# quantscious/finmlkit

Hardware: AMD Instinct MI355X
Metric: ticks/sec aggregated to bars (higher is better)
Workload: dtype f64

## Files before the change

### finmlkit_amd/csrc/fmk_median.h

```cpp
#pragma once
#include <math.h>

#include "fmk_common.h"
#include "fmk_dpp.h"

template <bool AF64> struct MedKey;
template <> struct MedKey<false> {
    typedef uint32_t K;
    static constexpr int BITS = 32;
    static constexpr K MAXK = 0xFFFFFFFFu;
    static constexpr K KEY_NEG_INF = 0x007FFFFFu;
    static constexpr K KEY_POS_INF = 0xFF800000u;
    __device__ static __forceinline__ K tokey(K u) { return (u & 0x80000000u) ? ~u : (u | 0x80000000u); }
    __device__ static __forceinline__ K load(const void *p, int64_t j) { return tokey(((const uint32_t *)p)[j]); }
    __device__ static __forceinline__ double value(K k)
    {
        uint32_t u = (k & 0x80000000u) ? (k & 0x7FFFFFFFu) : ~k;
        return (double)__uint_as_float(u);
    }
};
template <> struct MedKey<true> {
    typedef uint64_t K;
    static constexpr int BITS = 64;
    static constexpr K MAXK = 0xFFFFFFFFFFFFFFFFull;
// ... 21 lines not shown
__device__ __forceinline__ K med_wave_umax(K v)
{
#pragma unroll
    for (int o = 32; o > 0; o >>= 1) { K w = __shfl_xor(v, o, 64); v = w > v ? w : v; }
    return v;
}

template <typename K>
__device__ __forceinline__ K med_bitonic64(K v, int lane)
{
#pragma unroll
    for (int k = 2; k <= 64; k <<= 1) {
#pragma unroll
        for (int j = k >> 1; j > 0; j >>= 1) {
            K w = __shfl_xor(v, j, 64);
            bool up = (lane & k) == 0;
            bool lower = (lane & j) == 0;
            K mn = w < v ? w : v, mx = w < v ? v : w;
            v = (lower == up) ? mn : mx;
        }
    }
    return v;
}

template <bool AF64, int NREG, bool EXACT = false>
struct MedBar {
    typedef MedKey<AF64> MK;
    typedef typename MK::K K;
    K key[NREG > 0 ? NREG : 1];
    const void *amount;
    int64_t start, cnt;
    int lane;

    __device__ __forceinline__ void load_all()
    {
        if constexpr (NREG > 0) {
            K raw[NREG];
#pragma unroll
            for (int r = 0; r < NREG; ++r) {
                const int64_t j = (int64_t)r * 64 + lane;
                raw[r] = 0;
                if (j < cnt) raw[r] = ((const K *)amount)[start + j];
            }
#pragma unroll
            for (int r = 0; r < NREG; ++r) asm volatile("" : "+v"(raw[r]));
#pragma unroll
            for (int r = 0; r < NREG; ++r) {
                const int64_t j = (int64_t)r * 64 + lane;
                key[r] = j < cnt ? MK::tokey(raw[r]) : MK::MAXK;
            }
        }
    }
    __device__ __forceinline__ bool maybe_invalid(int r) const { return !EXACT || r == NREG - 1; }
    __device__ __forceinline__ void minmax(K &mn, K &mx)
    {
        K a = MK::MAXK, b = 0;
        if constexpr (NREG > 0) {
#pragma unroll
            for (int r = 0; r < NREG; ++r) {
                const K k = key[r];
                a = k < a ? k : a;
                if (maybe_invalid(r)) b = (k != MK::MAXK && k > b) ? k : b;
                else b = k > b ? k : b;
            }
        } else {
            for (int64_t j = lane; j < cnt; j += 64) {
                K k = MK::load(amount, start + j);
                a = k < a ? k : a;
                b = k > b ? k : b;
            }
        }
        mn = med_wave_umin<K>(a);
        mx = med_wave_umax<K>(b);
    }
    __device__ __forceinline__ int64_t count_le(K pivot)
    {
        if constexpr (NREG > 0) {
            int c = 0;
#pragma unroll
            for (int r = 0; r < NREG; ++r) c += med_popc(key[r] <= pivot);
            return c;
        } else {
            int64_t c = 0;
            for (int64_t j = lane; j < cnt; j += 64) c += MK::load(amount, start + j) <= pivot;
            return fmk_wave_sum(c);
        }
    }
    __device__ __forceinline__ void split(K pivot, K &below, K &above)
    {
        K a = 0, b = MK::MAXK;
        if constexpr (NREG > 0) {
#pragma unroll
            for (int r = 0; r < NREG; ++r) {
                const K k = key[r];
                a = (k <= pivot && k > a) ? k : a;
                b = (k > pivot && k < b) ? k : b;
            }
        } else {
            for (int64_t j = lane; j < cnt; j += 64) {
                K k = MK::load(amount, start + j);
                a = (k <= pivot && k > a) ? k : a;
                b = (k > pivot && k < b) ? k : b;
            }
        }
        below = med_wave_umax<K>(a);
        above = med_wave_umin<K>(b);
    }
    __device__ __forceinline__ void inside_minmax(K lo, K hi, K &mn, K &mx)
    {
        K a = MK::MAXK, b = 0;
#pragma unroll
        for (int r = 0; r < (NREG > 0 ? NREG : 1); ++r) {
            const K k = key[r];
            const bool in = k > lo && k <= hi;
            a = (in && k < a) ? k : a;
            b = (in && k > b) ? k : b;
        }
        mn = med_wave_umin<K>(a);
        mx = med_wave_umax<K>(b);
    }
    __device__ __forceinline__ void compact(K lo, K hi, K *buf)
    {
        int base = 0;
        if constexpr (NREG > 0) {
#pragma unroll
            for (int r = 0; r < NREG; ++r) {
                K k = key[r];
                bool in = k > lo && k <= hi;
                uint64_t m = __ballot(in);
                int pos = base + __builtin_amdgcn_mbcnt_hi((uint32_t)(m >> 32), __builtin_amdgcn_mbcnt_lo((uint32_t)m, 0));
                if (in) buf[pos] = k;
                base += __popcll(m);
            }
        } else {
            for (int64_t j0 = 0; j0 < cnt; j0 += 64) {
                int64_t j = j0 + lane;
                K k = j < cnt ? MK::load(amount, start + j) : MK::MAXK;
                bool in = j < cnt && k > lo && k <= hi;
                uint64_t m = __ballot(in);
                int pos = base + __builtin_amdgcn_mbcnt_hi((uint32_t)(m >> 32), __builtin_amdgcn_mbcnt_lo((uint32_t)m, 0));
                if (in) buf[pos] = k;
                base += __popcll(m);
            }
        }
    }
};

template <bool AF64, int NREG, bool EXACT, bool SNAP = false>
__device__ __forceinline__ bool med_rank_pair(MedBar<AF64, NREG, EXACT> &bar, typename MedKey<AF64>::K *buf,
                                              int64_t k1, int64_t k2, typename MedKey<AF64>::K &v1,
                                              typename MedKey<AF64>::K &v2)
{
    typedef MedKey<AF64> MK;
    typedef typename MK::K K;
    const int lane = bar.lane;
    const int64_t cnt = bar.cnt;
    K mn, mx;
    bar.minmax(mn, mx);
    if (mn < MK::KEY_NEG_INF || mx > MK::KEY_POS_INF) return false;
    K lo = mn - 1, hi = mx;
    int64_t clo = 0, chi = cnt;
    for (int nstep = 0;; ++nstep) {
        if constexpr (SNAP && NREG > 0) {
            if (chi - clo > 64 && hi - lo > 1 && (nstep == 10 || nstep == 16 || nstep == 22)) {
                K mn_in, mx_in;
                bar.inside_minmax(lo, hi, mn_in, mx_in);
                hi = mx_in;
                lo = (mn_in == mx_in ? mx_in : mn_in) - 1;
                continue;
            }
        }
        if (chi - clo <= 64) {
            buf[lane] = MK::MAXK;
            __builtin_amdgcn_wave_barrier();
            bar.compact(lo, hi, buf);
            __builtin_amdgcn_wave_barrier();
            K v = med_bitonic64<K>(buf[lane], lane);
            __builtin_amdgcn_wave_barrier();
            v1 = __shfl(v, (int)(k1 - clo), 64);
            v2 = __shfl(v, (int)(k2 - clo), 64);
            break;
        }
        if (hi - lo == 1) { v1 = v2 = hi; break; }
        K pivot = lo + ((hi - lo) >> 1);
        int64_t c = bar.count_le(pivot);
        if (c > k2) { hi = pivot; chi = c; }
        else if (c <= k1) { lo = pivot; clo = c; }
        else {
            bar.split(pivot, v1, v2);
            break;
        }
    }
    return true;
}

template <bool AF64, int NREG, bool EXACT, bool SNAP = false>
__device__ __forceinline__ double med_search(MedBar<AF64, NREG, EXACT> &bar, typename MedKey<AF64>::K *buf)
{
    typedef MedKey<AF64> MK;
    typename MK::K v1, v2;
    const int64_t cnt = bar.cnt;
    if (!med_rank_pair<AF64, NREG, EXACT, SNAP>(bar, buf, (cnt - 1) >> 1, cnt >> 1, v1, v2)) return NAN;
    return (cnt & 1) ? MK::value(v1) : (MK::value(v1) + MK::value(v2)) / 2.0;
}

template <bool AF64, int NREG>
__device__ __forceinline__ double med_select(const void *amount, int64_t start, int64_t cnt, int lane,
                                             typename MedKey<AF64>::K *buf)
{
    MedBar<AF64, NREG, false> bar;
    bar.amount = amount; bar.start = start; bar.cnt = cnt; bar.lane = lane;
    bar.load_all();
    return med_search<AF64, NREG, false>(bar, buf);
}

#define MED_SEL_BITS 11
#define MED_SEL_BINS (1 << MED_SEL_BITS)
template <bool AF64, int THREADS>
__device__ __forceinline__ void med_block_select(const void *__restrict__ amount, int64_t start, int64_t cnt, int64_t rank0,
                                                 int64_t rank1, typename MedKey<AF64>::K &k1, typename MedKey<AF64>::K &k2,
                                                 bool &any_nan)
{
    typedef MedKey<AF64> MK;
    typedef typename MK::K K;
    constexpr int D = (MK::BITS + MED_SEL_BITS - 1) / MED_SEL_BITS;
    constexpr int PER = MED_SEL_BINS / THREADS;
    constexpr int NW = THREADS / 64;
    __shared__ unsigned hist[2][MED_SEL_BINS];
    __shared__ K s_prefix[2];
    __shared__ int64_t s_rank[2];
    __shared__ unsigned s_wsum[2][NW];
    __shared__ int s_nan;
    const int tid = threadIdx.x, lane = fmk_lane(), w = tid >> 6;
    __syncthreads();
    if (tid == 0) { s_prefix[0] = 0; s_prefix[1] = 0; s_rank[0] = rank0; s_rank[1] = rank1; s_nan = 0; }
    bool nan = false;
#pragma unroll 1
    for (int p = 0; p < D; ++p) {
#pragma unroll
        for (int q = 0; q < PER; ++q) { hist[0][tid + q * THREADS] = 0; hist[1][tid + q * THREADS] = 0; }
        __syncthreads();
        const K pre0 = s_prefix[0], pre1 = s_prefix[1];
        const int64_t rk0 = s_rank[0], rk1 = s_rank[1];
        const bool same = pre0 == pre1;
        const int rest = MK::BITS - MED_SEL_BITS * (p + 1);
        const int shift = rest > 0 ? rest : 0;
        const int width = rest >= 0 ? MED_SEL_BITS : MED_SEL_BITS + rest;
        const unsigned mask = (1u << width) - 1u;
        for (int64_t j = tid; j < cnt; j += THREADS) {
            const K k = MK::load(amount, start + j);
            if (p == 0) nan |= k < MK::KEY_NEG_INF || k > MK::KEY_POS_INF;
            const K hi = p == 0 ? (K)0 : (K)(k >> (shift + width));
            const unsigned d = (unsigned)(k >> shift) & mask;
            if (hi == pre0) atomicAdd(&hist[0][d], 1u);
            if (!same && hi == pre1) atomicAdd(&hist[1][d], 1u);
        }
        __syncthreads();
#pragma unroll
        for (int t = 0; t < 2; ++t) {
            const unsigned *hh = hist[same ? 0 : t];
            unsigned h[PER], tot = 0;
#pragma unroll
            for (int q = 0; q < PER; ++q) { h[q] = hh[tid * PER + q]; tot += h[q]; }
            unsigned inc = tot;
#pragma unroll
            for (int o = 1; o < 64; o <<= 1) { const unsigned v = __shfl_up(inc, o, 64); if (lane >= o) inc += v; }
            if (lane == 63) s_wsum[t][w] = inc;
            __syncthreads();
            unsigned base = 0;
            for (int k = 0; k < w; ++k) base += s_wsum[t][k];
            int64_t cum = (int64_t)base + inc - tot;
            const int64_t rk = t == 0 ? rk0 : rk1;
#pragma unroll
            for (int q = 0; q < PER; ++q) {
                if (cum <= rk && rk < cum + h[q]) {
                    s_prefix[t] = (K)(((t == 0 ? pre0 : pre1) << width) | (K)(tid * PER + q));
                    s_rank[t] = rk - cum;
                }
                cum += h[q];
            }
        }
        __syncthreads();
    }
    if (nan) s_nan = 1;
    __syncthreads();
    k1 = s_prefix[0]; k2 = s_prefix[1]; any_nan = s_nan != 0;
}

struct FuMed {
    uint32_t lo, hi;
    uint32_t width;
    int have;
};

__device__ __forceinline__ uint32_t fu_wave_umin(uint32_t v)
{
    return (uint32_t)fmk_dpp_reduce((int)(v ^ 0x80000000u), (int)0x7FFFFFFF, FmkOpMin()) ^ 0x80000000u;
}
__device__ __forceinline__ uint32_t fu_wave_umax(uint32_t v)
{
    return (uint32_t)fmk_dpp_reduce((int)(v ^ 0x80000000u), (int)0x80000000, FmkOpMax()) ^ 0x80000000u;
}

template <int R>
__device__ __forceinline__ double fu_median(const uint32_t (&key)[R], int cnt, int lane, bool maybe_nan, FuMed &med, uint32_t *buf)
{
    typedef MedKey<false> MK;
    const int k1 = (cnt - 1) >> 1, k2 = cnt >> 1;
    uint32_t lo = 0, hi = 0;
    int clo = 0, chi = cnt;
    bool inside = false;
    if (med.have && !maybe_nan) {
        int c1 = 0, c2 = 0;
#pragma unroll
        for (int i = 0; i < R; ++i) {
            c1 += med_popc(key[i] <= med.lo);
            c2 += med_popc(key[i] <= med.hi);
        }
        if (c1 <= k1 && k2 < c2) {
            inside = true; lo = med.lo; hi = med.hi; clo = c1; chi = c2;
            const int nc = c2 - c1;
            if (nc > 144) med.width -= med.width >> 2;
            else if (nc < 80) med.width += (med.width >> 2) + 1;
        }
    }
    if (!inside) {
        uint32_t a = MK::MAXK, bmax = 0;
#pragma unroll
        for (int i = 0; i < R; ++i) {
            const uint32_t k = key[i];
            a = k < a ? k : a;
            bmax = (k != MK::MAXK && k > bmax) ? k : bmax;
        }
        const uint32_t mn = fu_wave_umin(a), mx = fu_wave_umax(bmax);
        if (mn < MK::KEY_NEG_INF || mx > MK::KEY_POS_INF) { med.have = 0; return NAN; }
        lo = mn - 1; hi = mx; clo = 0; chi = cnt;
    }
    uint32_t v1 = 0, v2 = 0;
    bool found = false;
    while (chi - clo > 64) {
        if (hi - lo == 1) { v1 = v2 = hi; found = true; break; }
        const uint32_t pivot = lo + ((hi - lo) >> 1);
        int c = 0;
#pragma unroll
        for (int i = 0; i < R; ++i) c += med_popc(key[i] <= pivot);
        if (c > k2) { hi = pivot; chi = c; }
        else if (c <= k1) { lo = pivot; clo = c; }
        else {
            uint32_t a = 0, bb = MK::MAXK;
#pragma unroll
            for (int i = 0; i < R; ++i) {
                const uint32_t k = key[i];
                a = (k <= pivot && k > a) ? k : a;
                bb = (k > pivot && k < bb) ? k : bb;
            }
            v1 = fu_wave_umax(a); v2 = fu_wave_umin(bb);
            found = true;
            break;
        }
    }
    uint32_t cmin = 0, cmax = 0;
    if (!found) {
        buf[lane] = MK::MAXK;
        __builtin_amdgcn_wave_barrier();
        int base = 0;
#pragma unroll
        for (int i = 0; i < R; ++i) {
            const uint32_t k = key[i];
            const bool in = k > lo && k <= hi;
            const uint64_t m = __ballot(in);
            const int pos = base + (int)__builtin_amdgcn_mbcnt_hi((uint32_t)(m >> 32), __builtin_amdgcn_mbcnt_lo((uint32_t)m, 0));
            if (in) buf[pos] = k;
            base += __popcll(m);
        }
        __builtin_amdgcn_wave_barrier();
        const uint32_t c0 = buf[lane];
        __builtin_amdgcn_wave_barrier();
        if (!inside) {
            cmin = fu_wave_umin(c0);
            cmax = fu_wave_umax(lane < chi - clo ? c0 : 0u);
        }
        for (;;) {
            if (hi - lo == 1) { v1 = v2 = hi; break; }
            const uint32_t pivot = lo + ((hi - lo) >> 1);
            const int c = clo + med_popc(c0 <= pivot);
            if (c > k2) hi = pivot;
            else if (c <= k1) lo = pivot;
            else {
                v1 = fu_wave_umax(c0 <= pivot ? c0 : 0u);
                v2 = fu_wave_umin(c0 > pivot ? c0 : MK::MAXK);
                break;
            }
        }
    }
    if (!inside) {
        if (found) med.width = 64;
        else {
            const uint32_t wl = v1 - cmin, wh = cmax - v2;
            med.width = wl > wh ? wl : wh;
        }
        med.have = 1;
    }
    med.lo = v1 > med.width + 1 ? v1 - med.width - 1 : 0;
    med.hi = v2 < 0xFFFFFFFEu - med.width ? v2 + med.width : 0xFFFFFFFEu;
    return (cnt & 1) ? MK::value(v1) : (MK::value(v1) + MK::value(v2)) / 2.0;
}
```

### finmlkit_amd/csrc/fmk_ohlcv.hip

```cpp
#include <math.h>
#include <stdlib.h>

#include <utility>

#include "fmk_bars.h"
#include "fmk_common.h"
#include "fmk_dpp.h"
#include "fmk_f32tie.h"
#include "fmk_median.h"

#define FMK_SMALL_NCH 21
#define FMK_PACKED_MAX_MEAN 64

struct OhlcvOut {
    double *open, *high, *low, *close;
    float *vol;
    double *vwap;
    int64_t *trades;
    double *median;
    unsigned long long *vol_redo;
};

__device__ __forceinline__ void ohlcv_empty(const OhlcvOut &o, int64_t b, const double *price, int64_t e, int64_t n)
{
// ... 75 lines not shown
    if (go && *go == 0) return;
    __shared__ double s_red[4][OH_WIDE_THREADS / 64];
    __shared__ int s_ncand;
    __shared__ int64_t s_below[OH_WIDE_THREADS / 64];
    __shared__ int s_nan;
    const int tid = threadIdx.x, lane = fmk_lane(), w = tid >> 6;
    const int64_t n_list = list[0];
    for (int64_t q = blockIdx.x; q < n_list; q += gridDim.x) {
        const int64_t b = list[1 + q], s = ci[b], e = ci[b + 1], start = s + 1;
        double hi = -INFINITY, lo = INFINITY, tv = 0.0, td = 0.0;
        uint32_t blo = 0, bhi = 0;
        int64_t below = 0;
        bool nan = false;
        uint32_t *mycand = nullptr;
        int cap = 0;
        if constexpr (MED) {
            blo = brk[4 * q]; bhi = brk[4 * q + 1];
            mycand = cand + ((start - base) >> 2);
            cap = (int)((e - s) >> 2);
            if (tid == 0) { s_ncand = 0; s_nan = 0; }
            __syncthreads();
        }
        auto med_tick = [&](int64_t jj, bool in_bar) {
            if constexpr (MED) {
                const uint32_t raw = in_bar ? ((const uint32_t *)amount)[jj] : 0u;
                const uint32_t k = MedKey<false>::tokey(raw);
                nan |= in_bar && (k < MedKey<false>::KEY_NEG_INF || k > MedKey<false>::KEY_POS_INF);
                below += (in_bar && k < blo) ? 1 : 0;
                const bool inb = in_bar && k >= blo && k <= bhi;
                const uint64_t m = __ballot(inb);
                if (m) {
                    int base = 0;
                    if (lane == (int)__builtin_ctzll(m)) base = atomicAdd(&s_ncand, (int)__popcll(m));
                    base = __builtin_amdgcn_readlane(base, (int)__builtin_ctzll(m));
                    const int pos = base + (int)__builtin_amdgcn_mbcnt_hi((uint32_t)(m >> 32), __builtin_amdgcn_mbcnt_lo((uint32_t)m, 0));
                    if (inb && pos < cap) mycand[pos] = raw;
                }
            }
        };
        int64_t j = start + tid;
        for (; j + 3 * OH_WIDE_THREADS <= e; j += 4 * OH_WIDE_THREADS) {
            const double p0 = price[j], p1 = price[j + OH_WIDE_THREADS], p2 = price[j + 2 * OH_WIDE_THREADS],
                         p3 = price[j + 3 * OH_WIDE_THREADS];
            const double a0 = fmk_amt<AF64>(amount, j), a1 = fmk_amt<AF64>(amount, j + OH_WIDE_THREADS),
                         a2 = fmk_amt<AF64>(amount, j + 2 * OH_WIDE_THREADS), a3 = fmk_amt<AF64>(amount, j + 3 * OH_WIDE_THREADS);
            hi = fmax(fmax(hi, p0), fmax(p1, fmax(p2, p3)));
            lo = fmin(fmin(lo, p0), fmin(p1, fmin(p2, p3)));
            tv += a0; td += p0 * a0;
            tv += a1; td += p1 * a1;
            tv += a2; td += p2 * a2;
            tv += a3; td += p3 * a3;
            med_tick(j, true); med_tick(j + OH_WIDE_THREADS, true); med_tick(j + 2 * OH_WIDE_THREADS, true);
            med_tick(j + 3 * OH_WIDE_THREADS, true);
        }
        for (; j - tid <= e; j += OH_WIDE_THREADS) {
            const bool in_bar = j <= e;
            const int64_t jc = in_bar ? j : e;
            const double p0 = price[jc], a0 = in_bar ? fmk_amt<AF64>(amount, jc) : 0.0;
            hi = fmax(hi, p0);
            lo = fmin(lo, p0);
            tv += a0; td += in_bar ? p0 * a0 : 0.0;
            med_tick(jc, in_bar);
        }
        hi = fmk_dpp_reduce(hi, (double)-INFINITY, FmkOpMax());
        lo = fmk_dpp_reduce(lo, (double)INFINITY, FmkOpMin());
        tv = fmk_dpp_reduce(tv, 0.0, FmkOpAdd());
        td = fmk_dpp_reduce(td, 0.0, FmkOpAdd());
        if constexpr (MED) {
            below = fmk_dpp_reduce(below, (int64_t)0, FmkOpAdd());
            if (lane == 0) s_below[w] = below;
            if (__ballot(nan) != 0 && lane == 0) s_nan = 1;
        }
        if (lane == 0) { s_red[0][w] = hi; s_red[1][w] = lo; s_red[2][w] = tv; s_red[3][w] = td; }
        __syncthreads();
        if constexpr (MED) {
            if (tid == 0) {
                int64_t bl = 0;
                for (int k = 0; k < OH_WIDE_THREADS / 64; ++k) bl += s_below[k];
                res[3 * q] = bl; res[3 * q + 1] = s_ncand; res[3 * q + 2] = s_nan;
            }
        }
        if (w == 0) {
            hi = s_red[0][0]; lo = s_red[1][0]; tv = s_red[2][0]; td = s_red[3][0];
            for (int k = 1; k < OH_WIDE_THREADS / 64; ++k) {
                hi = fmax(hi, s_red[0][k]); lo = fmin(lo, s_red[1][k]); tv += s_red[2][k]; td += s_red[3][k];
            }
            ohlcv_finish<AF64>(o, b, price, start, e, hi, lo, tv, td, lane, true);
        }
        __syncthreads();
    }
}


struct OhlBracket { uint32_t blo, bhi; int ok; int pad; };
struct OhlCount { int64_t below; int64_t ncand; int64_t nan; };

__device__ __forceinline__ int ohl_stride(int64_t cnt) { return cnt <= 65536 ? 16 : (cnt <= ((int64_t)1 << 21) ? 64 : 256); }

__global__ __launch_bounds__(256) void k_bar_med_sample(const float *__restrict__ amount, const int64_t *__restrict__ ci,
                                                        const int64_t *__restrict__ list, const int *__restrict__ go,
                                                        float *__restrict__ samp, OhlBracket *__restrict__ brk, float g_scale,
                                                        int64_t base)
{
    if (go && *go == 0) return;
    const int64_t n_list = list[0];
    for (int64_t q = blockIdx.x; q < n_list; q += gridDim.x) {
        const int64_t b = list[1 + q], s0 = ci[b], e = ci[b + 1], start = s0 + 1, cnt = e - s0;
        const int stride = ohl_stride(cnt);
        const int64_t ns = cnt / stride;
        float *mine = samp + ((start - base) >> 4);
        for (int64_t j = threadIdx.x; j < ns; j += 256) mine[j] = amount[start + j * stride];
        __syncthreads();
        const int g = (int)(1.9f * g_scale * sqrtf((float)ns)) + 4;
        const int64_t r_lo = ns / 2 - g > 0 ? ns / 2 - g : 0, r_hi = ns / 2 + g < ns - 1 ? ns / 2 + g : ns - 1;
        uint32_t klo, khi;
        bool any_nan;
        med_block_select<false, 256>(mine, 0, ns, r_lo, r_hi, klo, khi, any_nan);
        if (threadIdx.x == 0) brk[q] = OhlBracket{klo, khi, any_nan ? 0 : 1, 0};
        __syncthreads();
    }
}

__global__ __launch_bounds__(256) void k_bar_med_finish(const int64_t *__restrict__ ci, const int64_t *__restrict__ list,
                                                        const int *__restrict__ go, const uint32_t *__restrict__ cand,
                                                        const OhlCount *__restrict__ res, int64_t *__restrict__ fallback,
                                                        double *__restrict__ o_median, int64_t base)
{
    if (go && *go == 0) return;
    typedef MedKey<false> MK;
    const int64_t n_list = list[0];
    for (int64_t q = blockIdx.x; q < n_list; q += gridDim.x) {
        const int64_t b = list[1 + q], s0 = ci[b], e = ci[b + 1], start = s0 + 1, cnt = e - s0;
        const OhlCount r = res[q];
        const int64_t k1 = (cnt - 1) >> 1, k2 = cnt >> 1, cap = cnt >> 2;
        if (r.nan) { if (threadIdx.x == 0) o_median[b] = NAN; continue; }
        if (!(r.below <= k1 && k2 < r.below + r.ncand && r.ncand <= cap)) {
            if (threadIdx.x == 0) fallback[1 + atomicAdd((unsigned long long *)fallback, 1ULL)] = b;
            continue;
        }
        uint32_t v1, v2;
        bool any_nan;
        med_block_select<false, 256>(cand + ((start - base) >> 2), 0, r.ncand, k1 - r.below, k2 - r.below, v1, v2, any_nan);
        if (threadIdx.x == 0) o_median[b] = (cnt & 1) ? MK::value(v1) : (MK::value(v1) + MK::value(v2)) / 2.0;
        __syncthreads();
    }
}

int fmk_median_long_list_launch(fmk_ctx *ctx, const void *d_amount, const int64_t *d_close_idx, const int64_t *d_list, double *d_median);

__global__ __launch_bounds__(256) void k_list_span(const int64_t *__restrict__ ci, const int64_t *__restrict__ list, int64_t *__restrict__ out)
{
    __shared__ long long s_lo, s_hi;
    if (threadIdx.x == 0) { s_lo = INT64_MAX; s_hi = 0; }
    __syncthreads();
    const int64_t n_list = list[0];
    long long lo = INT64_MAX, hi = 0;
    for (int64_t q = threadIdx.x; q < n_list; q += 256) {
        const int64_t b = list[1 + q];
        const long long s = ci[b] + 1, e = ci[b + 1] + 1;
        lo = s < lo ? s : lo;
        hi = e > hi ? e : hi;
    }
    atomicMin(&s_lo, lo);
    atomicMax(&s_hi, hi);
    __syncthreads();
    if (threadIdx.x == 0) { out[0] = n_list; out[1] = n_list ? s_lo : 0; out[2] = n_list ? s_hi : 0; }
}

template <bool AF64>
static int oh_wide_launch(fmk_ctx *ctx, const double *p, const void *a, const int64_t *ci, int64_t nb, int64_t n, const int *go,
                          const OhlcvOut &o, int *median_done = nullptr, int64_t wide_min = OH_WIDE_MIN)
{
    int64_t *list = nullptr;
    FMK_TRY(fmk_long_bar_list(ctx, ci, nb, n, wide_min, go, &list));
    if constexpr (!AF64) {
        if (o.median && median_done) {
            const int64_t cap = n / wide_min + 2;
            int64_t base = 0, span = n;
            if (!ctx->enqueue_only) {
                int64_t *d_span = ctx->d_mail->ohlcv.span, h_span[3];
                k_list_span<<<1, 256, 0, ctx->stream>>>(ci, list, d_span);
                FMK_LAUNCH_CHECK(ctx);
                FMK_TRY(fmk_read_back(ctx, h_span, d_span, sizeof h_span));
                if (h_span[0] == 0) {
                    FMK_TRY(fmk_free(ctx, list));
                    *median_done = 1;
                    return FMK_OK;
                }
                base = h_span[1] & ~(int64_t)15;
                span = h_span[2] - base;
            }
            float *samp = nullptr;
            uint32_t *cand = nullptr;
            OhlBracket *brk = nullptr;
            int64_t *res = nullptr, *fallback = nullptr;
            int rc = fmk_alloc(ctx, (size_t)((span >> 4) + 64) * 4, (void **)&samp);
            if (rc == FMK_OK) rc = fmk_alloc(ctx, (size_t)((span >> 2) + 64) * 4, (void **)&cand);
            if (rc == FMK_OK) rc = fmk_alloc(ctx, (size_t)cap * sizeof(OhlBracket), (void **)&brk);
            if (rc == FMK_OK) rc = fmk_alloc(ctx, (size_t)cap * 3 * 8, (void **)&res);
            if (rc == FMK_OK) rc = fmk_alloc(ctx, (size_t)(cap + 1) * 8, (void **)&fallback);
            const bool have_scratch = rc == FMK_OK;
            hipError_t le = hipSuccess;
            if (have_scratch) le = hipMemsetAsync(fallback, 0, 8, ctx->stream);
            if (have_scratch && le == hipSuccess) {
                const char *gv = getenv("FMK_WIDE_MED_GSCALE");
                k_bar_med_sample<<<(unsigned)(ctx->n_cu * 4), 256, 0, ctx->stream>>>((const float *)a, ci, list, go, samp, brk,
                                                                                   gv ? (float)atof(gv) : 1.0f, base);
                k_bar_ohlcv_wide<false, true><<<(unsigned)(ctx->n_cu * 2), OH_WIDE_THREADS, 0, ctx->stream>>>(
                    p, a, ci, list, go, o, (const uint32_t *)brk, cand, res, base);
                k_bar_med_finish<<<(unsigned)(ctx->n_cu * 4), 256, 0, ctx->stream>>>(ci, list, go, cand, (const OhlCount *)res, fallback,
                                                                                   o.median, base);
                le = hipGetLastError();
                rc = FMK_OK;
                if (le == hipSuccess) rc = fmk_median_long_list_launch(ctx, a, ci, fallback, o.median);
            }
            if (samp) (void)fmk_free(ctx, samp);
            if (cand) (void)fmk_free(ctx, cand);
            if (brk) (void)fmk_free(ctx, brk);
            if (res) (void)fmk_free(ctx, res);
            if (fallback) (void)fmk_free(ctx, fallback);
            if (have_scratch) {
                (void)fmk_free(ctx, list);
                FMK_TRY(rc);
                FMK_HIP(ctx, le);
                *median_done = 1;
                return FMK_OK;
            }
            if (rc != FMK_E_NOMEM) { (void)fmk_free(ctx, list); FMK_TRY(rc); }
        }
    }
    k_bar_ohlcv_wide<AF64><<<(unsigned)(ctx->n_cu * 2), OH_WIDE_THREADS, 0, ctx->stream>>>(p, a, ci, list, go, o);
    const hipError_t le = hipGetLastError();
    FMK_TRY(fmk_free(ctx, list));
    FMK_HIP(ctx, le);
    return FMK_OK;
}

template <bool AF64>
__global__ __launch_bounds__(256) void k_bar_ohlcv(const double *__restrict__ price,
                                                   const void *__restrict__ amount,
                                                   const int64_t *__restrict__ ci, int64_t nb, int64_t n,
                                                   int64_t min_cnt, const int *__restrict__ go, OhlcvOut o,
                                                   int64_t skip_lo = 0, int64_t skip_hi = 0)
{
    if (go && *go == 0) return;
    const int lane = fmk_lane();
    const int wpb = blockDim.x >> 6;
    const int64_t wave0 = (int64_t)blockIdx.x * wpb + fmk_uniform((int)(threadIdx.x >> 6));
    const int64_t nwaves = (int64_t)gridDim.x * wpb;
    auto do_bar = [&](int64_t b, int64_t s, int64_t e) {
        if (e <= s) {
            if (lane == 0) ohlcv_empty(o, b, price, e, n);
            return;
        }
        if (e - s > OH_WIDE_MIN) return;
        if (e - s > skip_lo && e - s <= skip_hi) return;
        const int64_t start = s + 1;
        double hi = -INFINITY, lo = INFINITY, tv = 0.0, td = 0.0;
        int64_t j = start + lane;
        for (; j + 192 <= e; j += 256) {
            double p0 = price[j], p1 = price[j + 64], p2 = price[j + 128], p3 = price[j + 192];
            double a0 = fmk_amt<AF64>(amount, j), a1 = fmk_amt<AF64>(amount, j + 64);
            double a2 = fmk_amt<AF64>(amount, j + 128), a3 = fmk_amt<AF64>(amount, j + 192);
            hi = fmax(fmax(hi, p0), fmax(p1, fmax(p2, p3)));
            lo = fmin(fmin(lo, p0), fmin(p1, fmin(p2, p3)));
            tv += a0; td += p0 * a0;
            tv += a1; td += p1 * a1;
            tv += a2; td += p2 * a2;
            tv += a3; td += p3 * a3;
        }
        for (; j <= e; j += 64) {
            double p0 = price[j];
            double a0 = fmk_amt<AF64>(amount, j);
            hi = fmax(hi, p0);
            lo = fmin(lo, p0);
            tv += a0; td += p0 * a0;
        }
        ohlcv_finish<AF64>(o, b, price, start, e, hi, lo, tv, td, lane);
    };
    if (min_cnt > 0) { fmk_for_long_bars(ci, nb, min_cnt, wave0, nwaves, lane, do_bar); return; }
    for (int64_t b = wave0; b < nb; b += nwaves) do_bar(b, fmk_uniform(ci[b]), fmk_uniform(ci[b + 1]));
}

template <bool AF64, int NCH, bool EXACT, bool MEDIAN>
__device__ __forceinline__ void small_bar(const double *__restrict__ price, const void *__restrict__ amount,
                                          int64_t b, int64_t start, int64_t e, int64_t cnt, int lane,
                                          typename MedKey<AF64>::K *buf, const OhlcvOut &o)
{
    typedef MedKey<AF64> MK;
    typedef typename MK::K K;
    const double *pb = price + start;
    const K *ab = (const K *)amount + start;
    const unsigned last = (unsigned)(cnt - 1);
    double p[NCH];
    K araw[NCH];
#pragma unroll
    for (int c = 0; c < NCH; ++c) {
        unsigned idx = (unsigned)(c * 64 + lane);
        if (!EXACT || c == NCH - 1) idx = idx < last ? idx : last;
        p[c] = pb[idx];
        araw[c] = ab[idx];
    }
    double hi = -INFINITY, lo = INFINITY, tv = 0.0, td = 0.0;
    MedBar<AF64, NCH, EXACT> bar;
#pragma unroll
    for (int c = 0; c < NCH; ++c) {
        double a;
        if constexpr (AF64) a = __longlong_as_double((long long)araw[c]);
        else a = (double)__uint_as_float(araw[c]);
        hi = fmax(hi, p[c]);
        lo = fmin(lo, p[c]);
        const double pa = p[c] * a;
        if (!EXACT || c == NCH - 1) {
            const bool valid = (unsigned)(c * 64 + lane) <= last;
            tv += valid ? a : 0.0;
            td += valid ? pa : 0.0;
            if constexpr (MEDIAN) bar.key[c] = valid ? MK::tokey(araw[c]) : MK::MAXK;
        } else {
            tv += a;
            td += pa;
            if constexpr (MEDIAN) bar.key[c] = MK::tokey(araw[c]);
        }
    }
    ohlcv_finish<AF64>(o, b, price, start, e, hi, lo, tv, td, lane);
    if constexpr (MEDIAN) {
        bar.amount = amount; bar.start = start; bar.cnt = cnt; bar.lane = lane;
        const double m = med_search<AF64, NCH, EXACT>(bar, buf);
        if (lane == 0) o.median[b] = m;
    }
}

template <bool AF64, bool MEDIAN, int MAXNCH = FMK_SMALL_NCH>
__global__ __launch_bounds__(256, (MAXNCH <= 4 ? 8 : MAXNCH <= 10 ? 6 : 4)) void k_bar_ohlcv_small(const double *__restrict__ price,
                                                            const void *__restrict__ amount,
                                                            const int64_t *__restrict__ ci, int64_t nb, int64_t n,
                                                            int *__restrict__ saw_long, OhlcvOut o)
{
    typedef typename MedKey<AF64>::K K;
    __shared__ K sbuf[4][64];
    const int lane = fmk_lane();
    const int wib = fmk_uniform((int)(threadIdx.x >> 6));
    const int wpb = blockDim.x >> 6;
    const int64_t wave0 = (int64_t)blockIdx.x * wpb + wib;
    const int64_t nwaves = (int64_t)gridDim.x * wpb;
    K *buf = sbuf[wib];
    for (int64_t b = wave0; b < nb; b += nwaves) {
        const int64_t s = fmk_uniform(ci[b]);
        const int64_t e = fmk_uniform(ci[b + 1]);
        const int64_t cnt = e - s;
        if (cnt > 64 * MAXNCH) {
            if (lane == 0) fmk_raise(saw_long);
            continue;
        }
        if (cnt <= 0) {
            if (lane == 0) ohlcv_empty(o, b, price, e, n);
            continue;
        }
        const int64_t start = s + 1;
        const int nch = (int)((cnt + 63) >> 6);
        if constexpr (MAXNCH <= 4) {
            switch (nch) {
            case 1: small_bar<AF64, 1, true, MEDIAN>(price, amount, b, start, e, cnt, lane, buf, o); break;
            case 2: small_bar<AF64, 2, true, MEDIAN>(price, amount, b, start, e, cnt, lane, buf, o); break;
            case 3: small_bar<AF64, 3, true, MEDIAN>(price, amount, b, start, e, cnt, lane, buf, o); break;
            default: small_bar<AF64, 4, true, MEDIAN>(price, amount, b, start, e, cnt, lane, buf, o); break;
            }
        } else if constexpr (MAXNCH <= 10) {
            switch (nch) {
            case 1: small_bar<AF64, 1, true, MEDIAN>(price, amount, b, start, e, cnt, lane, buf, o); break;
            case 2: small_bar<AF64, 2, true, MEDIAN>(price, amount, b, start, e, cnt, lane, buf, o); break;
            case 3: small_bar<AF64, 3, true, MEDIAN>(price, amount, b, start, e, cnt, lane, buf, o); break;
            case 4: small_bar<AF64, 4, true, MEDIAN>(price, amount, b, start, e, cnt, lane, buf, o); break;
            case 5: small_bar<AF64, 5, true, MEDIAN>(price, amount, b, start, e, cnt, lane, buf, o); break;
            case 6: small_bar<AF64, 6, true, MEDIAN>(price, amount, b, start, e, cnt, lane, buf, o); break;
            case 7: small_bar<AF64, 7, true, MEDIAN>(price, amount, b, start, e, cnt, lane, buf, o); break;
            case 8: small_bar<AF64, 8, true, MEDIAN>(price, amount, b, start, e, cnt, lane, buf, o); break;
            case 9: small_bar<AF64, 9, true, MEDIAN>(price, amount, b, start, e, cnt, lane, buf, o); break;
            default: small_bar<AF64, 10, true, MEDIAN>(price, amount, b, start, e, cnt, lane, buf, o); break;
            }
        } else {
            switch (nch) {
            case 11: small_bar<AF64, 11, true, MEDIAN>(price, amount, b, start, e, cnt, lane, buf, o); break;
            case 12: small_bar<AF64, 12, true, MEDIAN>(price, amount, b, start, e, cnt, lane, buf, o); break;
            case 13: small_bar<AF64, 13, true, MEDIAN>(price, amount, b, start, e, cnt, lane, buf, o); break;
            case 14: small_bar<AF64, 14, true, MEDIAN>(price, amount, b, start, e, cnt, lane, buf, o); break;
            case 15: small_bar<AF64, 15, true, MEDIAN>(price, amount, b, start, e, cnt, lane, buf, o); break;
            case 16: small_bar<AF64, 16, true, MEDIAN>(price, amount, b, start, e, cnt, lane, buf, o); break;
            case 17: small_bar<AF64, 17, true, MEDIAN>(price, amount, b, start, e, cnt, lane, buf, o); break;
            case 18: small_bar<AF64, 18, true, MEDIAN>(price, amount, b, start, e, cnt, lane, buf, o); break;
            case 19: small_bar<AF64, 19, true, MEDIAN>(price, amount, b, start, e, cnt, lane, buf, o); break;
            case 20: small_bar<AF64, 20, true, MEDIAN>(price, amount, b, start, e, cnt, lane, buf, o); break;
            case 21: small_bar<AF64, 21, true, MEDIAN>(price, amount, b, start, e, cnt, lane, buf, o); break;
            default:
                if (nch <= 1) small_bar<AF64, 1, true, MEDIAN>(price, amount, b, start, e, cnt, lane, buf, o);
                else if (nch <= 4) small_bar<AF64, 4, false, MEDIAN>(price, amount, b, start, e, cnt, lane, buf, o);
                else if (nch <= 10) small_bar<AF64, 10, false, MEDIAN>(price, amount, b, start, e, cnt, lane, buf, o);
                else small_bar<AF64, 16, false, MEDIAN>(price, amount, b, start, e, cnt, lane, buf, o);
            }
        }
    }
}

struct TbFuse {
    const int64_t *ts;
    int64_t e0, d;
    int64_t t_first, t_last;
    int64_t *clock, *idx;
};


template <int NCH>
__device__ __forceinline__ void median_bar(const void *__restrict__ amount, int64_t b, int64_t start, int64_t cnt, int lane,
                                           uint32_t *buf, double *__restrict__ o_median, FuMed &med)
{
    typedef MedKey<false> MK;
    const uint32_t *ab = (const uint32_t *)amount + start;
    const unsigned last = (unsigned)(cnt - 1);
    uint32_t key[NCH];
    bool nan = false;
#pragma unroll
    for (int c = 0; c < NCH; ++c) {
        unsigned idx = (unsigned)(c * 64 + lane);
        if (c == NCH - 1) idx = idx < last ? idx : last;
        const uint32_t raw = ab[idx];
        nan |= (raw & 0x7FFFFFFFu) > 0x7F800000u;
        key[c] = (c < NCH - 1 || (unsigned)(c * 64 + lane) <= last) ? MK::tokey(raw) : MK::MAXK;
    }
    const bool any_nan = __ballot(nan) != 0;
    double m;
    if (any_nan) { m = NAN; med.have = 0; }
    else m = fu_median<NCH>(key, (int)cnt, lane, false, med, buf);
    if (lane == 0) o_median[b] = m;
}

__global__ __launch_bounds__(256) void k_bar_median_small(const float *__restrict__ amount, const int64_t *__restrict__ ci,
                                                          int64_t nb, int *__restrict__ saw_long, double *__restrict__ o_median)
{
    __shared__ uint32_t sbuf[4][64];
    const int lane = fmk_lane();
    const int wib = fmk_uniform((int)(threadIdx.x >> 6));
    const int64_t wave0 = (int64_t)blockIdx.x * 4 + wib;
    const int64_t nwaves = (int64_t)gridDim.x * 4;
    uint32_t *buf = sbuf[wib];
    FuMed med;
    med.lo = med.hi = 0; med.width = 64; med.have = 0;
    for (int64_t b = wave0; b < nb; b += nwaves) {
        const int64_t s = fmk_uniform(ci[b]);
        const int64_t e = fmk_uniform(ci[b + 1]);
        const int64_t cnt = e - s;
        if (cnt > 64 * FMK_SMALL_NCH) {
            if (lane == 0) fmk_raise(saw_long);
            continue;
        }
        if (cnt <= 0) { if (lane == 0) o_median[b] = 0.0; continue; }
        const int64_t start = s + 1;
        switch ((int)((cnt + 63) >> 6)) {
#define FMK_MB(N) case N: median_bar<N>(amount, b, start, cnt, lane, buf, o_median, med); break;
            FMK_MB(1) FMK_MB(2) FMK_MB(3) FMK_MB(4) FMK_MB(5) FMK_MB(6) FMK_MB(7) FMK_MB(8) FMK_MB(9) FMK_MB(10) FMK_MB(11)
            FMK_MB(12) FMK_MB(13) FMK_MB(14) FMK_MB(15) FMK_MB(16) FMK_MB(17) FMK_MB(18) FMK_MB(19) FMK_MB(20)
#undef FMK_MB
        default: median_bar<21>(amount, b, start, cnt, lane, buf, o_median, med); break;
        }
    }
}

int fmk_median_small_launch(fmk_ctx *ctx, const float *d_amount, const int64_t *d_close_idx, int64_t nb, double *d_median,
                            int64_t n_ticks)
{
    int *saw_long = &ctx->d_mail->ohlcv.saw_long;
    FMK_HIP(ctx, hipMemsetAsync(saw_long, 0, sizeof(int), ctx->stream));
    int64_t blocks = fmk_ceil_div(nb, 4);
    const int64_t cap = (int64_t)ctx->n_cu * 64;
    if (blocks > cap) blocks = cap;
    if (blocks < 1) blocks = 1;
    k_bar_median_small<<<(unsigned)blocks, 256, 0, ctx->stream>>>(d_amount, d_close_idx, nb, saw_long, d_median);
    FMK_LAUNCH_CHECK(ctx);
    return fmk_median_launch(ctx, d_amount, 0, d_close_idx, nb, 64 * FMK_SMALL_NCH, saw_long, d_median, n_ticks);
}


template <bool MEDIAN, int N, int K, int NR>
__device__ __forceinline__ void lb_block(const double *tp, const uint32_t *ta, int off, int L, int Lmax, int zero_at, double &hi, double &lo,
                                         double (&lv)[3], double (&ld)[3], double &tv, double &td, uint32_t (&r)[NR])
{
    typedef MedKey<false> MK;
    constexpr int j0 = 8 * K;
    double cv = 0.0, cd = 0.0;
    if (j0 < Lmax) {
        double p[8];
        uint32_t raw[8];
#pragma unroll
        for (int q = 0; q < 8; ++q) {
            const int at = j0 + q < L ? off + j0 + q : zero_at;
            p[q] = tp[at];
            raw[q] = ta[at];
        }
        double xv[8], xd[8];
#pragma unroll
        for (int q = 0; q < 8; ++q) {
            const bool in = j0 + q < L;
            const double a = (double)__uint_as_float(raw[q]);
            if (in) {
                hi = p[q] > hi ? p[q] : hi;
                lo = p[q] < lo ? p[q] : lo;
            }
            xv[q] = a;
            xd[q] = p[q] * a;
            if constexpr (MEDIAN) r[j0 + q] = in ? MK::tokey(raw[q]) : MK::MAXK;
        }
        cv = ((xv[0] + xv[1]) + (xv[2] + xv[3])) + ((xv[4] + xv[5]) + (xv[6] + xv[7]));
        cd = ((xd[0] + xd[1]) + (xd[2] + xd[3])) + ((xd[4] + xd[5]) + (xd[6] + xd[7]));
    } else if constexpr (MEDIAN) {
#pragma unroll
        for (int q = 0; q < 8; ++q) r[j0 + q] = MK::MAXK;
    }
    constexpr int NB = N / 8;
    if constexpr ((K & 1) == 0 && NB > 1) { lv[0] = cv; ld[0] = cd; }
    else {
        if constexpr (NB > 1) { cv = lv[0] + cv; cd = ld[0] + cd; }
        if constexpr ((K & 2) == 0 && NB > 2) { lv[1] = cv; ld[1] = cd; }
        else {
            if constexpr (NB > 2) { cv = lv[1] + cv; cd = ld[1] + cd; }
            if constexpr ((K & 4) == 0 && NB > 4) { lv[2] = cv; ld[2] = cd; }
            else {
                if constexpr (NB > 4) { cv = lv[2] + cv; cd = ld[2] + cd; }
                tv = cv; td = cd;
            }
        }
    }
    __builtin_amdgcn_sched_barrier(0);
    asm volatile("" ::: "memory");
    if constexpr (K + 1 < NB) lb_block<MEDIAN, N, K + 1, NR>(tp, ta, off, L, Lmax, zero_at, hi, lo, lv, ld, tv, td, r);
}

template <bool MEDIAN, int N>
__device__ __forceinline__ void lb_bar(const double *tp, const uint32_t *ta, int off, int L, int zero_at, double &hi, double &lo,
                                       double &tv, double &td, double &med)
{
    typedef MedKey<false> MK;
    uint32_t r[MEDIAN ? N : 1];
    double lv[3] = {0.0, 0.0, 0.0}, ld[3] = {0.0, 0.0, 0.0};
    const int Lmax = fmk_dpp_reduce(L, 0, FmkOpMax());
    lb_block<MEDIAN, N, 0, (MEDIAN ? N : 1)>(tp, ta, off, L, Lmax, zero_at, hi, lo, lv, ld, tv, td, r);
    if constexpr (MEDIAN) {
        fmk_lane_sort<N>(r);
        const uint32_t v1 = fmk_lane_pick<N>(r, (L - 1) >> 1), v2 = fmk_lane_pick<N>(r, L >> 1);
        const uint32_t kmx = fmk_lane_pick<N>(r, L > 0 ? L - 1 : 0), kmn = r[0];
        if (kmn < MK::KEY_NEG_INF || kmx > MK::KEY_POS_INF) med = NAN;
        else med = (L & 1) ? MK::value(v1) : (MK::value(v1) + MK::value(v2)) / 2.0;
    }
}

template <bool MEDIAN, int LB_TILE>
__global__ __launch_bounds__(128) void k_bar_ohlcv_lanes(const double *__restrict__ price, const float *__restrict__ amount,
                                                         const int64_t *__restrict__ ci, int64_t nb, int64_t n,
                                                         int *__restrict__ saw_long, OhlcvOut o)
{
    __shared__ double s_p[2][LB_TILE + 2];
    __shared__ uint32_t s_a[2][LB_TILE + 2];
    __shared__ int64_t s_ci[2][66];
    const int lane = fmk_lane();
    const int w = fmk_uniform((int)(threadIdx.x >> 6));
    double *tp = s_p[w];
    uint32_t *ta = s_a[w];
    if (lane == 0) { tp[LB_TILE] = 0.0; ta[LB_TILE] = 0u; }
    const int64_t ngroups = (nb + 63) >> 6;
    const int64_t nwaves = (int64_t)gridDim.x * 2;
    for (int64_t g = (int64_t)blockIdx.x * 2 + w; g < ngroups; g += nwaves) {
        const int64_t B0 = g * 64;
        const int nbg = fmk_lane_group_load(s_ci[w], ci, nb, B0, lane);
        int bl = 0;
        while (bl < nbg) {
            const int64_t s0 = s_ci[w][bl];
            const int idx = bl + 1 + lane;
            const bool valid = idx <= nbg;
            const int64_t e_l = valid ? s_ci[w][idx] : INT64_MAX;
            const int64_t s_l = valid ? s_ci[w][idx - 1] : 0;
            const int m = __popcll(__ballot(valid && e_l - s0 <= LB_TILE));
            if (m == 0) {
                if (lane == 0) fmk_raise(saw_long);
                bl += 1;
                continue;
            }
            const int ntick = (int)(s_ci[w][bl + m] - s0);
            __builtin_amdgcn_wave_barrier();
            const double *gp = price + s0 + 1;
            const uint32_t *ga = (const uint32_t *)amount + s0 + 1;
#pragma unroll 4
            for (int j = lane; j < ntick; j += 64) {
                tp[j] = gp[j];
                ta[j] = ga[j];
            }
            __builtin_amdgcn_wave_barrier();
            const bool owner = lane < m;
            const int L = owner ? (int)(e_l - s_l) : 0;
            const bool mine = owner && L > 0 && L <= 64;
            const int off = mine ? (int)(s_l - s0) : 0;
            const uint64_t longer = __ballot(owner && L > 64);
            if (longer && lane == 0) fmk_raise(saw_long);
            const int Lw = mine ? L : 0;
            const bool any_gt32 = __ballot(Lw > 32) != 0;
            const double first = ntick > 0 ? tp[off] : 0.0;
            double hi = first, lo = first, tv = 0.0, td = 0.0;
            double med = 0.0;
            if (any_gt32) lb_bar<MEDIAN, 64>(tp, ta, off, Lw, LB_TILE, hi, lo, tv, td, med);
            else lb_bar<MEDIAN, 32>(tp, ta, off, Lw, LB_TILE, hi, lo, tv, td, med);
            if (owner) {
                const int64_t b = B0 + bl + lane;
                if (mine) {
                    o.open[b] = first;
                    o.close[b] = tp[off + L - 1];
                    o.high[b] = hi;
                    o.low[b] = lo;
                    o.vol[b] = (float)tv;
                    o.vwap[b] = tv > 0.0 ? td / tv : 0.0;
                    o.trades[b] = L;
                    if constexpr (MEDIAN) o.median[b] = med;
                } else if (L == 0) {
                    ohlcv_empty(o, b, price, e_l, n);
                }
            }
            bl += m;
        }
    }
}


#define OHR_WAVES 4
#define OHR_CAND 16
template <int LPB> __device__ __forceinline__ double ohr_sum(double v)
{
    v += fmk_dpp<DPP_XOR1, 0xF>(v, v);
    v += fmk_dpp<DPP_XOR2, 0xF>(v, v);
    if constexpr (LPB >= 8) v += fmk_dpp<DPP_HALF_MIRROR, 0xF>(v, v);
    if constexpr (LPB == 16) v += fmk_dpp<DPP_MIRROR, 0xF>(v, v);
    return v;
}
template <int LPB> __device__ __forceinline__ double ohr_max(double v)
{
    v = fmax(v, fmk_dpp<DPP_XOR1, 0xF>(v, v));
    v = fmax(v, fmk_dpp<DPP_XOR2, 0xF>(v, v));
    if constexpr (LPB >= 8) v = fmax(v, fmk_dpp<DPP_HALF_MIRROR, 0xF>(v, v));
// ... 773 lines not shown
```

Baseline: 429.2 billion.

## Replace small-bar median search with register bisection plus LDS compaction

```diff
diff --git a/finmlkit_amd/csrc/fmk_median.h b/finmlkit_amd/csrc/fmk_median.h
--- a/finmlkit_amd/csrc/fmk_median.h
+++ b/finmlkit_amd/csrc/fmk_median.h
@@ -347,6 +347,99 @@
     return (uint32_t)fmk_dpp_reduce((int)(v ^ 0x80000000u), (int)0x80000000, FmkOpMax()) ^ 0x80000000u;
 }
 
+__device__ __forceinline__ uint64_t fu_wave_umin(uint64_t v)
+{
+    return (uint64_t)fmk_dpp_reduce((int64_t)(v ^ 0x8000000000000000ull), (int64_t)0x7FFFFFFFFFFFFFFFll, FmkOpMin()) ^ 0x8000000000000000ull;
+}
+__device__ __forceinline__ uint64_t fu_wave_umax(uint64_t v)
+{
+    return (uint64_t)fmk_dpp_reduce((int64_t)(v ^ 0x8000000000000000ull), (int64_t)0x8000000000000000ull, FmkOpMax()) ^ 0x8000000000000000ull;
+}
+
+template <bool AF64, int NCH, bool EXACT>
+__device__ __forceinline__ double med_search_small(const typename MedKey<AF64>::K (&key)[NCH], int cnt, int lane,
+                                                   typename MedKey<AF64>::K *buf)
+{
+    typedef MedKey<AF64> MK;
+    typedef typename MK::K K;
+    const int k1 = (cnt - 1) >> 1, k2 = cnt >> 1;
+    K a = MK::MAXK, b = 0;
+#pragma unroll
+    for (int r = 0; r < NCH; ++r) {
+        const K k = key[r];
+        a = k < a ? k : a;
+        if (!EXACT || r == NCH - 1) b = (k != MK::MAXK && k > b) ? k : b;
+        else b = k > b ? k : b;
+    }
+    const K mn = fu_wave_umin(a), mx = fu_wave_umax(b);
+    if (mn < MK::KEY_NEG_INF || mx > MK::KEY_POS_INF) return NAN;
+    K lo = mn - 1, hi = mx;
+    int clo = 0, chi = cnt;
+    K v1 = 0, v2 = 0;
+    bool found = false;
+    while (chi - clo > 64) {
+        if (hi - lo == 1) { v1 = v2 = hi; found = true; break; }
+        const K pivot = lo + ((hi - lo) >> 1);
+        int c = 0;
+#pragma unroll
+        for (int r = 0; r < NCH; ++r) c += med_popc(key[r] <= pivot);
+        if (c > k2) { hi = pivot; chi = c; }
+        else if (c <= k1) { lo = pivot; clo = c; }
+        else {
+            K s = 0, t = MK::MAXK;
+#pragma unroll
+            for (int r = 0; r < NCH; ++r) {
+                const K k = key[r];
+                s = (k <= pivot && k > s) ? k : s;
+                t = (k > pivot && k < t) ? k : t;
+            }
+            v1 = fu_wave_umax(s); v2 = fu_wave_umin(t);
+            found = true;
+            break;
+        }
+    }
+    if (!found) {
+        const K lo1 = lo + 1, span = hi - lo;
+        int n = 0;
+#pragma unroll
+        for (int r = 0; r < NCH; ++r) n += (K)(key[r] - lo1) < span;
+        int pos = fmk_dpp_iscan(n, 0, FmkOpAdd()) - n;
+        buf[lane] = MK::MAXK;
+        __builtin_amdgcn_wave_barrier();
+#pragma unroll
+        for (int r = 0; r < NCH; ++r) {
+            const K k = key[r];
+            const bool in = (K)(k - lo1) < span;
+            buf[in ? pos : 64 + lane] = k;
+            pos += in;
+        }
+        __builtin_amdgcn_wave_barrier();
+        const K c0 = buf[lane];
+        __builtin_amdgcn_wave_barrier();
+        const int base = clo;
+        for (;;) {
+            if (chi - clo <= 2) {
+                const bool in = (K)(c0 - (lo + 1)) < (K)(hi - lo);
+                const K cmn = fu_wave_umin(in ? c0 : MK::MAXK), cmx = fu_wave_umax(in ? c0 : (K)0);
+                v1 = k1 == clo ? cmn : cmx;
+                v2 = k2 == clo ? cmn : cmx;
+                break;
+            }
+            if (hi - lo == 1) { v1 = v2 = hi; break; }
+            const K pivot = lo + ((hi - lo) >> 1);
+            const int c = base + med_popc(c0 <= pivot);
+            if (c > k2) { hi = pivot; chi = c; }
+            else if (c <= k1) { lo = pivot; clo = c; }
+            else {
+                v1 = fu_wave_umax(c0 <= pivot ? c0 : (K)0);
+                v2 = fu_wave_umin(c0 > pivot ? c0 : MK::MAXK);
+                break;
+            }
+        }
+    }
+    return (cnt & 1) ? MK::value(v1) : (MK::value(v1) + MK::value(v2)) / 2.0;
+}
+
 template <int R>
 __device__ __forceinline__ double fu_median(const uint32_t (&key)[R], int cnt, int lane, bool maybe_nan, FuMed &med, uint32_t *buf)
 {
diff --git a/finmlkit_amd/csrc/fmk_ohlcv.hip b/finmlkit_amd/csrc/fmk_ohlcv.hip
--- a/finmlkit_amd/csrc/fmk_ohlcv.hip
+++ b/finmlkit_amd/csrc/fmk_ohlcv.hip
@@ -401,7 +401,7 @@
         araw[c] = ab[idx];
     }
     double hi = -INFINITY, lo = INFINITY, tv = 0.0, td = 0.0;
-    MedBar<AF64, NCH, EXACT> bar;
+    K key[MEDIAN ? NCH : 1];
 #pragma unroll
     for (int c = 0; c < NCH; ++c) {
         double a;
@@ -414,17 +414,16 @@
             const bool valid = (unsigned)(c * 64 + lane) <= last;
             tv += valid ? a : 0.0;
             td += valid ? pa : 0.0;
-            if constexpr (MEDIAN) bar.key[c] = valid ? MK::tokey(araw[c]) : MK::MAXK;
+            if constexpr (MEDIAN) key[c] = valid ? MK::tokey(araw[c]) : MK::MAXK;
         } else {
             tv += a;
             td += pa;
-            if constexpr (MEDIAN) bar.key[c] = MK::tokey(araw[c]);
+            if constexpr (MEDIAN) key[c] = MK::tokey(araw[c]);
         }
     }
     ohlcv_finish<AF64>(o, b, price, start, e, hi, lo, tv, td, lane);
     if constexpr (MEDIAN) {
-        bar.amount = amount; bar.start = start; bar.cnt = cnt; bar.lane = lane;
-        const double m = med_search<AF64, NCH, EXACT>(bar, buf);
+        const double m = med_search_small<AF64, NCH, EXACT>(key, (int)cnt, lane, buf);
         if (lane == 0) o.median[b] = m;
     }
 }
@@ -436,7 +435,7 @@
                                                             int *__restrict__ saw_long, OhlcvOut o)
 {
     typedef typename MedKey<AF64>::K K;
-    __shared__ K sbuf[4][64];
+    __shared__ K sbuf[4][128];
     const int lane = fmk_lane();
     const int wib = fmk_uniform((int)(threadIdx.x >> 6));
     const int wpb = blockDim.x >> 6;
```

New measurement: 432.1 billion, median of 2. About the same (+0.7%).
